# shanice-l/gdrnpp_bop2022

Hardware: AMD Instinct MI355X
Metric: ROIs/sec (GDRNPP fwd + PnP + depth refine), 256x256 crops (higher is better)
Workload: dtype f32

## Files before the change

gdrnpp_bop2022_amd/csrc/capi.hip:

```cpp
#include "gemm_split.hpp"
#include <cstring>
#include <atomic>
#include <mutex>

namespace gdrnpp {
static thread_local char g_err[512] = "";
void set_error(const char* fmt, ...) {
  va_list ap;
  va_start(ap, fmt);
  vsnprintf(g_err, sizeof(g_err), fmt, ap);
  va_end(ap);
}
void* shim_scratch(size_t bytes) {
  static thread_local void* block = nullptr;
  static thread_local size_t cap = 0;
  static thread_local int block_dev = -1;
  int dev = 0;
  hipError_t e = hipGetDevice(&dev);
  if (e != hipSuccess) { set_error("hipGetDevice: %s", hipGetErrorString(e)); return nullptr; }
  if (block && block_dev == dev && cap >= bytes) return block;
  if (block) { (void)hipFree(block); block = nullptr; cap = 0; }
  const size_t want = bytes < ((size_t)1 << 20) ? ((size_t)1 << 20) : bytes + (bytes >> 2);
  e = hipMalloc(&block, want);
  if (e != hipSuccess) { block = nullptr; set_error("hipMalloc(%zu): %s", want, hipGetErrorString(e)); return nullptr; }
  cap = want; block_dev = dev;
  return block;
}
int ensure_dynamic_lds(const void* kernel, int bytes) {
  struct Entry { const void* fn; int dev, bytes; };
  static std::mutex mu;
  static Entry table[128];
  static int n = 0;
  int dev = 0;
  GDRNPP_HIP_TRY(hipGetDevice(&dev));
  std::lock_guard<std::mutex> lock(mu);
  Entry* e = nullptr;
  for (int i = 0; i < n; ++i)
    if (table[i].fn == kernel && table[i].dev == dev) e = &table[i];
  if (e && e->bytes >= bytes) return 0;
  GDRNPP_HIP_TRY(hipFuncSetAttribute(kernel, hipFuncAttributeMaxDynamicSharedMemorySize, bytes));
  if (e) e->bytes = bytes;
  else if (n < 128) table[n++] = Entry{kernel, dev, bytes};
  return 0;
}
static std::atomic<int> g_opt_glds{1}, g_opt_mi4{-1}, g_opt_pipe{3}, g_opt_panel{4}, g_opt_big_tiles{256}, g_opt_dw_tile{-1}, g_opt_splitk_small{1}, g_opt_mlp_fused_pipe{1}, g_opt_dw_lds_w{1}, g_opt_dw_lds_pad{0}, g_opt_upconv_lowres{1}, g_opt_dw_specialise{1};
int option_split_gemm_glds() { return g_opt_glds; }
int option_split_gemm_pipe() { return g_opt_pipe; }
int option_split_gemm_mi4() { return g_opt_mi4; }
int option_split_gemm_panel() { return g_opt_panel; }
int option_split_gemm_big_tiles() { return g_opt_big_tiles; }
int option_dwconv_tile() { return g_opt_dw_tile; }
int option_splitk_small_tiles() { return g_opt_splitk_small; }
int option_mlp_fused_pipe() { return g_opt_mlp_fused_pipe; }
int option_dwconv_lds_w() { return g_opt_dw_lds_w; }
int option_dwconv_lds_pad() { return g_opt_dw_lds_pad; }
int option_dwconv_specialise() { return g_opt_dw_specialise; }
}

namespace {
template <int WIDTH>
__global__ void stream_read_kernel(const float* __restrict__ p, size_t n, float* __restrict__ out) {
  float acc = 0.f;
  const size_t stride = (size_t)gridDim.x * blockDim.x;
  if (WIDTH == 4) {
    const float4* q = reinterpret_cast<const float4*>(p);
    for (size_t i = (size_t)blockIdx.x * blockDim.x + threadIdx.x; i < n / 4; i += stride) {
      const float4 v = q[i];
      acc += (v.x + v.y) + (v.z + v.w);
    }
  } else {
    for (size_t i = (size_t)blockIdx.x * blockDim.x + threadIdx.x; i < n; i += stride) acc += p[i];
  }
  for (int off = 32; off >= 1; off >>= 1) acc += __shfl_xor(acc, off, 64);
  if ((threadIdx.x & 63) == 0) atomicAdd(out + blockIdx.x, acc);
}
__global__ void spin_kernel(long long ticks) {
  const long long t0 = wall_clock64();
  while (wall_clock64() - t0 < ticks) __builtin_amdgcn_s_sleep(8);
}
}

extern "C" {
int gdrnpp_debug_spin(int micros, void* stream) {
  GDRNPP_REQUIRE(micros >= 1 && micros <= 1000000, GDRNPP_EINVAL, "gdrnpp_debug_spin: micros must be in [1, 1000000]");
  int dev = 0, khz = 0;
  GDRNPP_HIP_TRY(hipGetDevice(&dev));
  GDRNPP_HIP_TRY(hipDeviceGetAttribute(&khz, hipDeviceAttributeWallClockRate, dev));
  if (khz <= 0) khz = 100000;
  hipLaunchKernelGGL(spin_kernel, dim3(1), dim3(64), 0, (hipStream_t)stream, (long long)micros * khz / 1000);
  return gdrnpp::check_launch("gdrnpp_debug_spin");
}
int gdrnpp_debug_stream_read(const float* p, size_t n, int lane_bytes, float* out_blocks, int blocks, void* stream) {
  GDRNPP_REQUIRE(p && out_blocks && n > 0 && blocks > 0 && (lane_bytes == 4 || lane_bytes == 16), GDRNPP_EINVAL,
                 "gdrnpp_debug_stream_read: bad arguments");
  if (lane_bytes == 16)
    hipLaunchKernelGGL(stream_read_kernel<4>, dim3(blocks), dim3(256), 0, (hipStream_t)stream, p, n, out_blocks);
  else
    hipLaunchKernelGGL(stream_read_kernel<1>, dim3(blocks), dim3(256), 0, (hipStream_t)stream, p, n, out_blocks);
  return gdrnpp::check_launch("gdrnpp_debug_stream_read");
}
int gdrnpp_copy_d2d(void* dst, const void* src, size_t bytes, void* stream) {
  if (bytes == 0) return 0;
  GDRNPP_REQUIRE(dst && src, GDRNPP_EINVAL, "gdrnpp_copy_d2d: null pointer");
  GDRNPP_HIP_TRY(hipMemcpyAsync(dst, src, bytes, hipMemcpyDeviceToDevice, (hipStream_t)stream));
  return 0;
}
int gdrnpp_set_option(const char* name, int value) {
  GDRNPP_REQUIRE(name, GDRNPP_EINVAL, "gdrnpp_set_option: null name");
  if (!strcmp(name, "split_gemm_glds")) { gdrnpp::g_opt_glds = value != 0; return 0; }
  if (!strcmp(name, "split_gemm_pipe")) { gdrnpp::g_opt_pipe = value == 3 ? 3 : (value != 0 ? 2 : 0); return 0; }
  if (!strcmp(name, "split_gemm_panel")) { gdrnpp::g_opt_panel = value < 2 ? 0 : (value > 64 ? 64 : value); return 0; }
  if (!strcmp(name, "split_gemm_big_tiles")) { gdrnpp::g_opt_big_tiles = value < 1 ? 1 : value; return 0; }
  if (!strcmp(name, "splitk_small_tiles")) { gdrnpp::g_opt_splitk_small = value != 0; return 0; }
  if (!strcmp(name, "dwconv_tile")) { gdrnpp::g_opt_dw_tile = (value >= 0 && value <= 2) ? value : -1; return 0; }
  if (!strcmp(name, "mlp_fused_pipe")) { gdrnpp::g_opt_mlp_fused_pipe = value != 0; return 0; }
  if (!strcmp(name, "dwconv_lds_w")) { gdrnpp::g_opt_dw_lds_w = value != 0; return 0; }
  if (!strcmp(name, "dwconv_specialise")) { gdrnpp::g_opt_dw_specialise = value != 0; return 0; }
  if (!strcmp(name, "dwconv_lds_pad")) { gdrnpp::g_opt_dw_lds_pad = value < 0 ? 0 : (value > 112 * 1024 ? 112 * 1024 : value); return 0; }
  if (!strcmp(name, "split_gemm_mi4")) { gdrnpp::g_opt_mi4 = value < 0 ? -1 : (value != 0); return 0; }
  if (!strcmp(name, "upconv_lowres")) { gdrnpp::g_opt_upconv_lowres = value != 0; return 0; }
  gdrnpp::set_error("gdrnpp_set_option: unknown option '%s'", name);
  return GDRNPP_EINVAL;
}
int gdrnpp_get_option(const char* name, int* value) {
  GDRNPP_REQUIRE(name && value, GDRNPP_EINVAL, "gdrnpp_get_option: null pointer");
  static const struct { const char* name; std::atomic<int>* opt; } table[] = {
      {"split_gemm_glds", &gdrnpp::g_opt_glds},       {"split_gemm_pipe", &gdrnpp::g_opt_pipe},
      {"split_gemm_panel", &gdrnpp::g_opt_panel},     {"split_gemm_big_tiles", &gdrnpp::g_opt_big_tiles},
      {"splitk_small_tiles", &gdrnpp::g_opt_splitk_small}, {"dwconv_tile", &gdrnpp::g_opt_dw_tile},
      {"mlp_fused_pipe", &gdrnpp::g_opt_mlp_fused_pipe}, {"dwconv_lds_w", &gdrnpp::g_opt_dw_lds_w},
      {"dwconv_lds_pad", &gdrnpp::g_opt_dw_lds_pad},  {"split_gemm_mi4", &gdrnpp::g_opt_mi4},
      {"upconv_lowres", &gdrnpp::g_opt_upconv_lowres}, {"dwconv_specialise", &gdrnpp::g_opt_dw_specialise}};
  for (const auto& e : table)
    if (!strcmp(name, e.name)) { *value = e.opt->load(); return 0; }
  gdrnpp::set_error("gdrnpp_get_option: unknown option '%s'", name);
  return GDRNPP_EINVAL;
}
int gdrnpp_version(void) { return 110;  }
const char* gdrnpp_last_error(void) { return gdrnpp::g_err; }
}
```

gdrnpp_bop2022_amd/csrc/common.hpp:

```cpp
#pragma once
#include <hip/hip_runtime.h>
#include <cstdio>
#include <cstdarg>
#include <cstdlib>
#include "../../include/gdrnpp_hip.h"

namespace gdrnpp {

void set_error(const char* fmt, ...);

inline int check_launch(const char* what) {
  hipError_t e = hipGetLastError();
  if (e != hipSuccess) {
    set_error("%s: %s", what, hipGetErrorString(e));
    return (int)e;
  }
  return 0;
}

#define GDRNPP_REQUIRE(cond, code, ...) \
  do {                                  \
    if (!(cond)) {                      \
      gdrnpp::set_error(__VA_ARGS__);   \
      return (code);                    \
    }                                   \
  } while (0)

#define GDRNPP_HIP_TRY(expr)                                        \
  do {                                                              \
    hipError_t _e = (expr);                                         \
    if (_e != hipSuccess) {                                         \
      gdrnpp::set_error("%s: %s", #expr, hipGetErrorString(_e));    \
      return (int)_e;                                               \
    }                                                               \
  } while (0)

constexpr int kWave = 64;

__device__ __forceinline__ float gelu_erf(float x) {
  const float u = fminf(fabsf(x), 5.9f);
  float q = -2.7721912374545354e-06f;
  q = fmaf(q, u, 3.862218727590516e-05f);
  q = fmaf(q, u, -0.00018255332543049008f);
  q = fmaf(q, u, -0.000145858692121692f);
  q = fmaf(q, u, 0.007075459696352482f);
  q = fmaf(q, u, -0.052505023777484894f);
  q = fmaf(q, u, -0.45920491218566895f);
  q = fmaf(q, u, -1.1511057615280151f);
  q = fmaf(q, u, -1.0f);
  const float r = fmaf(-u, __builtin_amdgcn_exp2f(q), fmaxf(x, 0.f));
  return x != x ? x : r;
}

void* shim_scratch(size_t bytes);
int ensure_dynamic_lds(const void* kernel, int bytes);

int option_split_gemm_glds();
int option_split_gemm_mi4();
int option_splitk_small_tiles();
int option_mlp_fused_pipe();
int option_dwconv_tile();
int option_dwconv_lds_w();
int option_dwconv_specialise();
int option_dwconv_lds_pad();

}
```

gdrnpp_bop2022_amd/csrc/gemm_split2_pipe.hip:

```cpp
#include "split2_common.hpp"

namespace {

using namespace gdrnpp::split2;

constexpr int NA = 3;
constexpr int A_STAGE_B = 256 * BK * 4;
constexpr int W2_TILE_SLOTS = 2 * KB * BN;
constexpr int W2_TILE_B = W2_TILE_SLOTS * 16;
constexpr int NB = 4;
constexpr int NJ = 4;
constexpr int LDS_BYTES = NA * A_STAGE_B + NB * W2_TILE_B;

__device__ int g_split2_range_word;

template <bool APRE>
struct HalfSplit2T {
  float x[APRE ? 1 : 8];
  unsigned h[4], l[4];

  template <int S>
  __device__ __forceinline__ void step() {
    if constexpr (APRE) {
    } else if constexpr (S < 2) {
      h[2 * S] = cvt_pk_f16(x[4 * S], x[4 * S + 1]);
      h[2 * S + 1] = cvt_pk_f16(x[4 * S + 2], x[4 * S + 3]);
    } else if constexpr (S < 6) {
      constexpr int p = S - 2;
      x[2 * p] = residual<0>(x[2 * p], h[p]);
      x[2 * p + 1] = residual<1>(x[2 * p + 1], h[p]);
    } else {
      constexpr int q = S - 6;
      l[2 * q] = cvt_pk_f16(x[4 * q], x[4 * q + 1]);
      l[2 * q + 1] = cvt_pk_f16(x[4 * q + 2], x[4 * q + 3]);
    }
  }
  __device__ __forceinline__ void load(const uint4* lds, int slot0, int slot1) {
    if constexpr (APRE) {
      const uint4 a = lds[slot0], b = lds[slot1];
      h[0] = a.x; h[1] = a.y; h[2] = a.z; h[3] = a.w;
      l[0] = b.x; l[1] = b.y; l[2] = b.z; l[3] = b.w;
    } else {
      const float4 a = __builtin_bit_cast(float4, lds[slot0]), b = __builtin_bit_cast(float4, lds[slot1]);
      x[0] = a.x; x[1] = a.y; x[2] = a.z; x[3] = a.w;
      x[4] = b.x; x[5] = b.y; x[6] = b.z; x[7] = b.w;
    }
  }
  template <int SPLIT>
  __device__ __forceinline__ f16x8 frag() const {
    const unsigned* s = SPLIT == 0 ? h : l;
    return __builtin_bit_cast(f16x8, make_uint4(s[0], s[1], s[2], s[3]));
  }
};

__global__ void pack_weight2_kernel(const float* __restrict__ W, uint4* __restrict__ packed, int N, int K) {
  const long i = (long)blockIdx.x * blockDim.x + threadIdx.x;
  const int kbs = K / 8;
  unsigned* trailer = reinterpret_cast<unsigned*>(packed + (size_t)(N / BN) * (K / BK) * W2_TILE_SLOTS);
  const int e = weight_exp(trailer[0]);
  const float sc = __builtin_ldexpf(1.f, e);
  if (i == 0) {
    trailer[1] = __float_as_uint(__builtin_ldexpf(1.f, -e));
    trailer[2] = __float_as_uint(sc);
    trailer[3] = 0u;
  }
  if (i >= (long)N * kbs) return;
  const int n = (int)(i / kbs), kb_g = (int)(i % kbs);
  const float4 v0 = *reinterpret_cast<const float4*>(W + (size_t)n * K + kb_g * 8);
  const float4 v1 = *reinterpret_cast<const float4*>(W + (size_t)n * K + kb_g * 8 + 4);
  const float x[8] = {v0.x * sc, v0.y * sc, v0.z * sc, v0.w * sc, v1.x * sc, v1.y * sc, v1.z * sc, v1.w * sc};
  unsigned h[4], l[4];
#pragma unroll
  for (int p = 0; p < 4; ++p) {
    h[p] = cvt_pk_f16(x[2 * p], x[2 * p + 1]);
    const f16x2 hv = __builtin_bit_cast(f16x2, h[p]);
    l[p] = cvt_pk_f16(x[2 * p] - (float)hv[0], x[2 * p + 1] - (float)hv[1]);
  }
  const int tn = n / BN, row = n % BN, tk = kb_g / KB, kb = kb_g % KB;
  uint4* img = packed + ((size_t)tn * (K / BK) + tk) * W2_TILE_SLOTS;
  img[(0 * KB + kb) * BN + row] = make_uint4(h[0], h[1], h[2], h[3]);
  img[(1 * KB + kb) * BN + row] = make_uint4(l[0], l[1], l[2], l[3]);
}

template <int EPI, int CONV, bool GNS, bool APRE = false>
__global__ __launch_bounds__(256, 2) void gemm_split2_pipe_kernel(const float* __restrict__ A, const uint4* __restrict__ Wp,
                                                                  const float* __restrict__ bias,
                                                                  const float* __restrict__ gamma,
                                                                  const float* __restrict__ resid, float* __restrict__ C,
                                                                  int M, int N, int K, ConvGeom cg, int panel, GnStats gn, int* range_flag, int c_rows) {
  static_assert(!APRE || CONV == 0, "f16x2-rows A: linear form only");
  using HalfSplit2 = HalfSplit2T<APRE>;
  constexpr int NS = 6 * NJ;
  constexpr int SB = 19;
  extern __shared__ uint4 smem[];
  const int tid = threadIdx.x, lane = tid & 63;
  const int wave = __builtin_amdgcn_readfirstlane(tid >> 6);
  const int ntn = N / BN;
  const TileMN tile = tile_coords(xcd_tile_id(), ntn, panel, M);
  const int tile_n = tile.n, m0 = tile.m * 256, n0 = tile_n * BN;
  const int nk = K / BK;
  const unsigned lds0 = lds_addr(smem);
  const float wsc = reinterpret_cast<const float*>(Wp + (size_t)(N / BN) * nk * W2_TILE_SLOTS)[1];

  const int prow = lane >> 2, pq = lane & 3;
  unsigned aoff[4];
  const float* ap[4];
  unsigned okmask[4];
  int cpt = 1;
#pragma unroll
  for (int c = 0; c < 4; ++c) {
    const int lrow = wave * 64 + c * 16 + prow;
    const int q = pq ^ ((lrow >> 2) & 3);
    const int arow = min(m0 + lrow, M - 1);
    if constexpr (CONV == 1) {
      const int img = arow / (cg.H * cg.W), pp = arow - img * (cg.H * cg.W);
      const int iy = pp / cg.W, ix = pp - iy * cg.W;
      ap[c] = A + ((size_t)arow) * cg.C + q * 4;
      unsigned mk = 0;
#pragma unroll
      for (int t = 0; t < 9; ++t) {
        const int dy = t / 3 - 1, dx = t % 3 - 1;
        if ((unsigned)(iy + dy) < (unsigned)cg.H && (unsigned)(ix + dx) < (unsigned)cg.W) mk |= 1u << t;
      }
      okmask[c] = mk;
      aoff[c] = 0;
    } else if constexpr (CONV == 2) {
      const int img = arow / (cg.OH * cg.OW), pp = arow - img * (cg.OH * cg.OW);
      const int iy = (pp / cg.OW) * cg.stride, ix = (pp % cg.OW) * cg.stride;
      ap[c] = A + (((size_t)img * cg.H + iy) * cg.W + ix) * cg.C + q * 4;
      const int ntaps = K / cg.C;
      unsigned mk = 0;
      for (int t = 0; t < ntaps; ++t) {
        const int ky = t / cg.KW, dy = ky - cg.pad, dx = t - ky * cg.KW - cg.pad;
        if ((unsigned)(iy + dy) < (unsigned)cg.H && (unsigned)(ix + dx) < (unsigned)cg.W) mk |= 1u << t;
      }
      okmask[c] = mk;
      aoff[c] = 0;
    } else {
      aoff[c] = (unsigned)arow * (unsigned)(K * 4) + (unsigned)(q * 16);
      ap[c] = nullptr;
      okmask[c] = 0;
    }
  }
  if constexpr (CONV) cpt = cg.C / BK;
  const int ntaps = CONV == 1 ? 9 : (CONV == 2 ? K / cg.C : 1), ckw = CONV == 1 ? 3 : cg.KW, cpad = CONV == 1 ? 1 : cg.pad;
  const unsigned boff = (unsigned)((wave * 2) * 64 + lane) * 16u;
  const char* const wbase = reinterpret_cast<const char*>(Wp + (size_t)tile_n * nk * W2_TILE_SLOTS);
  const unsigned ldsA = lds0 + (unsigned)(wave * 4) * 1024u;
  const unsigned ldsB = lds0 + (unsigned)(NA * A_STAGE_B) + (unsigned)(wave * 2) * 1024u;

  auto dma_a = [&](int kt, unsigned sb, auto cc) {
    constexpr int c = decltype(cc)::value;
    if constexpr (CONV) {
      GDRNPP_CONV_KTILE(kt, cpt, ntaps);
      const int c0 = chunk * BK;
      const int ky = tap / ckw, dy = ky - cpad, dx = tap - ky * ckw - cpad;
      const long off = ((long)dy * cg.W + dx) * cg.C + c0;
      const bool ok = (okmask[c] >> tap) & 1u;
      dma_v(ok ? (const void*)(ap[c] + off) : (const void*)g_zero_page, ldsA + sb + c * 1024u);
    } else {
      dma_s(aoff[c], reinterpret_cast<const char*>(A) + (size_t)kt * (BK * 4), ldsA + sb + c * 1024u);
    }
  };
  auto dma_b = [&](int kt, unsigned sb, auto cc) {
    constexpr int c = decltype(cc)::value;
    int wkt = kt;
    if constexpr (CONV) {
      GDRNPP_CONV_KTILE(kt, cpt, ntaps);
      wkt = tap * cpt + chunk;
    }
    dma_s(boff, wbase + ((size_t)wkt * W2_TILE_B + c * 1024), ldsB + sb + (unsigned)(c * 1024));
  };

  f32x16 acc[2][NJ];
#pragma unroll
  for (int i = 0; i < 2; ++i)
#pragma unroll
    for (int j = 0; j < NJ; ++j)
#pragma unroll
      for (int r = 0; r < 16; ++r) acc[i][j][r] = 0.f;

  const int frow = lane & 31, fk = lane >> 5;
  const int lrow0 = wave * 64 + frow, g0 = (lrow0 >> 2) & 3;
  const int aslot0 = 4 * lrow0 + ((2 * fk) ^ g0), aslot1 = 4 * lrow0 + ((2 * fk + 1) ^ g0);
  const uint4* const sA = smem;
  const uint4* const sBf = smem + NA * (A_STAGE_B / 16) + fk * BN + frow;

  auto load_half = [&](HalfSplit2& hs, int stage, int half) {
    hs.load(sA + stage * (A_STAGE_B / 16) + half * 128, aslot0, aslot1);
  };

  auto bslot = [](int P, int J) { return P * KB * BN + J * 32; };

  [[maybe_unused]] float ssq[4] = {0.f, 0.f, 0.f, 0.f};

  auto ktile = [&](int kt, HalfSplit2 (&cur)[2], HalfSplit2 (&nxt)[2], f16x8 (&fbL)[NJ], f16x8 (&fbH)[NJ], auto odd_, int sa1, int sa2,
                   int sa_wr) {
    constexpr int ODD = decltype(odd_)::value;
    const uint4* const b = sBf + (kt & 3) * (W2_TILE_B / 16);
    const uint4* const bn = sBf + ((kt + 1) & 3) * (W2_TILE_B / 16);
    const int kt_b = min(kt + 2, nk - 1), kt_a = min(kt + NA, nk - 1);
    const unsigned sb_wr = (unsigned)(((kt + 2) & 3) * W2_TILE_B), sa_wr_b = (unsigned)(sa_wr * A_STAGE_B);
    static_for<0, NS>([&](auto s_) {
      constexpr int S = decltype(s_)::value;
      constexpr int G = S / (2 * NJ), I = (S % (2 * NJ)) / NJ, J = S % NJ;
      const f16x8 fa = (G == 1) ? cur[I].template frag<1>() : cur[I].template frag<0>();
      const f16x8 fb = (G == 0) ? fbL[J] : fbH[J];
      acc[I][J] = __builtin_amdgcn_mfma_f32_32x32x16_f16(fa, fb, acc[I][J], 0, 0, 0);
#ifndef GDRNPP2_TIMING_NO_DMA
      if constexpr (S % 2 == 0 && S < 4) dma_b(kt_b, sb_wr, std::integral_constant<int, S / 2>{});
      if constexpr (S % 2 == 0 && S >= 4 && S < 12) dma_a(kt_a, sa_wr_b, std::integral_constant<int, (S - 4) / 2>{});
#endif
#ifndef GDRNPP2_TIMING_NO_BREAD
      if constexpr (S % 2 == 1 && S < NJ) {
        constexpr int j0 = S - 1;
        fbH[j0] = __builtin_bit_cast(f16x8, b[bslot(0, j0)]);
        fbH[j0 + 1] = __builtin_bit_cast(f16x8, b[bslot(0, j0 + 1)]);
      }
#endif
#ifndef GDRNPP2_NO_RANGE_CHECK
      {
        constexpr int rc[4] = {0, 2, 11, 12};
        if constexpr (S == rc[0]) { ssq[2] = sumsq2(cur[1].h[0], ssq[2]); ssq[3] = sumsq2(cur[1].h[1], ssq[3]); }
        if constexpr (S == rc[1]) { ssq[2] = sumsq2(cur[1].h[2], ssq[2]); ssq[3] = sumsq2(cur[1].h[3], ssq[3]); }
        if constexpr (S == rc[2]) { ssq[0] = sumsq2(cur[0].h[0], ssq[0]); ssq[1] = sumsq2(cur[0].h[1], ssq[1]); }
        if constexpr (S == rc[3]) { ssq[0] = sumsq2(cur[0].h[2], ssq[0]); ssq[1] = sumsq2(cur[0].h[3], ssq[1]); }
      }
#endif
      constexpr int S1 = 13;
      if constexpr (S == S1 - 4) load_half(nxt[1], sa1, 1);
#ifndef GDRNPP2_TIMING_NO_SPLIT
      if constexpr (S >= 3 && S < 11) nxt[0].template step<S - 3>();
      if constexpr (S >= S1 && S < S1 + 8) nxt[1].template step<S - S1>();
#else
      if constexpr (S == 3) { nxt[0].h[0] = __float_as_uint(nxt[0].x[0]); nxt[0].h[1] = __float_as_uint(nxt[0].x[1]); nxt[0].h[2] = __float_as_uint(nxt[0].x[2]); nxt[0].h[3] = __float_as_uint(nxt[0].x[3]);
                              nxt[0].l[0] = __float_as_uint(nxt[0].x[4]); nxt[0].l[1] = __float_as_uint(nxt[0].x[5]); nxt[0].l[2] = __float_as_uint(nxt[0].x[6]); nxt[0].l[3] = __float_as_uint(nxt[0].x[7]); }
      if constexpr (S == S1) { nxt[1].h[0] = __float_as_uint(nxt[1].x[0]); nxt[1].h[1] = __float_as_uint(nxt[1].x[1]); nxt[1].h[2] = __float_as_uint(nxt[1].x[2]); nxt[1].h[3] = __float_as_uint(nxt[1].x[3]);
                               nxt[1].l[0] = __float_as_uint(nxt[1].x[4]); nxt[1].l[1] = __float_as_uint(nxt[1].x[5]); nxt[1].l[2] = __float_as_uint(nxt[1].x[6]); nxt[1].l[3] = __float_as_uint(nxt[1].x[7]); }
#endif
      if constexpr (S == SB) {
#ifndef GDRNPP2_TIMING_NO_SYNC
        wait_vmcnt<4>();
        __builtin_amdgcn_s_waitcnt(0xc07f);
        if constexpr (ODD) __builtin_amdgcn_s_barrier();
#endif
      }
      constexpr int SL = APRE ? SB + 1 : SB;
#ifndef GDRNPP2_TIMING_NO_BREAD
      if constexpr (S > SL && S <= SL + NJ / 2) {
        constexpr int j0 = 2 * (S - SL - 1);
        fbL[j0] = __builtin_bit_cast(f16x8, bn[bslot(1, j0)]);
        fbL[j0 + 1] = __builtin_bit_cast(f16x8, bn[bslot(1, j0 + 1)]);
      }
#endif
      if constexpr (S == (APRE ? SB + 1 : SB + NJ / 2 + 1)) load_half(cur[0], sa2, 0);
      __builtin_amdgcn_sched_barrier(0);
    });
  };

  HalfSplit2 f0[2], f1[2];
  f16x8 fbL[NJ], fbH[NJ];
  static_for<0, 4>([&](auto c) { dma_a(0, 0u, c); });
  static_for<0, 2>([&](auto c) { dma_b(0, 0u, c); });
  static_for<0, 2>([&](auto c) { dma_b(min(1, nk - 1), (unsigned)W2_TILE_B, c); });
  static_for<0, 4>([&](auto c) { dma_a(min(1, nk - 1), (unsigned)A_STAGE_B, c); });
  static_for<0, 4>([&](auto c) { dma_a(min(2, nk - 1), 2u * A_STAGE_B, c); });
  wait_vmcnt<4>();
  __builtin_amdgcn_s_barrier();
  load_half(f0[0], 0, 0);
  load_half(f0[1], 0, 1);
  static_for<0, 8>([&](auto s) { f0[0].template step<decltype(s)::value>(); f0[1].template step<decltype(s)::value>(); });
#pragma unroll
  for (int j = 0; j < NJ; ++j) fbL[j] = __builtin_bit_cast(f16x8, sBf[bslot(1, j)]);
  load_half(f1[0], 1, 0);

  int sa = 0;
  for (int kt = 0; kt < nk; kt += 2) {
    const int sa1 = sa + 1 == NA ? 0 : sa + 1, sa2 = sa1 + 1 == NA ? 0 : sa1 + 1, sa3 = sa2 + 1 == NA ? 0 : sa2 + 1;
    ktile(kt, f0, f1, fbL, fbH, std::integral_constant<int, 0>{}, sa1, sa2, sa);
    ktile(kt + 1, f1, f0, fbL, fbH, std::integral_constant<int, 1>{}, sa2, sa3, sa1);
    sa = sa2;
  }
  wait_vmcnt<0>();
  __builtin_amdgcn_s_waitcnt(0xc07f);
  __builtin_amdgcn_s_barrier();

  bool bad = false;
#define EPI_TILES_M 2
#define EPI_HALVES (NJ / 2)
#define EPI_ACC(i, j) acc[i][j]
#define EPI_ROW0 m0 + wave * 64
#define EPI_COL0 n0
#define EPI_BIAS bias
#define EPI_STAGE smem
#define EPI_STAGE_BYTES (NA * A_STAGE_B)
#define EPI_SCALE wsc
#define EPI_GN gn
#define EPI_RANGE_BAD bad
#include "split_epilogue_body.hpp"
  bool small = false;
#ifndef GDRNPP2_NO_RANGE_CHECK
  {
    float s0 = ssq[0] + ssq[1], s1 = ssq[2] + ssq[3];
    s0 += __shfl_xor(s0, 32, 64);
    s1 += __shfl_xor(s1, 32, 64);
    const float thr = (float)K * 0x1p-8f;
    small = (s0 > 0.f && s0 < thr) || (s1 > 0.f && s1 < thr);
    bad |= !(s0 < __builtin_inff()) || !(s1 < __builtin_inff());
  }
#endif
  const int word = (__builtin_amdgcn_ballot_w64(bad) != 0 ? GDRNPP_SPLIT2_NONFINITE : 0) |
                   (__builtin_amdgcn_ballot_w64(small) != 0 ? GDRNPP_SPLIT2_SMALL_ROWS : 0);
  if (word && lane == 0) atomicOr(range_flag ? range_flag : &g_split2_range_word, word);
}

template <int EPI, int CONV, bool GNS, bool APRE = false>
int launch_kernel(const float* A, const uint4* Wp, const float* bias, const float* gamma, const float* resid, float* C, int M, int N,
                  int K, ConvGeom cg, int panel, GnStats gn, int* range_flag, hipStream_t st, const char* what, int c_rows = 0) {
  const int rc = gdrnpp::ensure_dynamic_lds((const void*)gemm_split2_pipe_kernel<EPI, CONV, GNS, APRE>, LDS_BYTES);
  if (rc) return rc;
  const long tiles = (long)((M + 255) / 256) * (N / BN);
  GDRNPP_REQUIRE(tiles < (1l << 30), GDRNPP_ELIMIT, "%s: grid too large", what);
  hipLaunchKernelGGL((gemm_split2_pipe_kernel<EPI, CONV, GNS, APRE>), dim3((unsigned)tiles), dim3(256), LDS_BYTES, st, A, Wp, bias, gamma,
                     resid, C, M, N, K, cg, panel, gn, range_flag, c_rows);
  return gdrnpp::check_launch(what);
}

template <int EPI, int CONV, bool GNS>
int launch_one(const float* A, const uint4* Wp, const float* bias, const float* gamma, const float* resid, float* C, int M, int N,
               int K, ConvGeom cg, int panel, GnStats gn, int* range_flag, hipStream_t st, const char* what, int a_rows = 0, int c_rows = 0) {
  if constexpr (CONV == 0 && EPI != EPI_BIAS) {
    if (a_rows) return launch_kernel<EPI, CONV, GNS, true>(A, Wp, bias, gamma, resid, C, M, N, K, cg, panel, gn, range_flag, st, what, c_rows);
  }
  return launch_kernel<EPI, CONV, GNS>(A, Wp, bias, gamma, resid, C, M, N, K, cg, panel, gn, range_flag, st, what, c_rows);
}

}

extern "C" size_t gdrnpp_pack_weight_f16x2_bytes(int N, int K) {
  return (N > 0 && K > 0) ? (size_t)N * (size_t)K * 4 + 16 : 0;
}

extern "C" int gdrnpp_pack_weight_f16x2(const float* W, void* packed, int N, int K, void* stream) {
  GDRNPP_REQUIRE(W && packed, GDRNPP_EINVAL, "gdrnpp_pack_weight_f16x2: null pointer");
  GDRNPP_REQUIRE(N > 0 && K > 0 && N % BN == 0 && K % 32 == 0, GDRNPP_ELIMIT,
                 "gdrnpp_pack_weight_f16x2: N=%d K=%d must be multiples of %d/32", N, K, BN);
  hipStream_t st = (hipStream_t)stream;
  unsigned* trailer = reinterpret_cast<unsigned*>(reinterpret_cast<uint4*>(packed) + (size_t)(N / BN) * (K / BK) * W2_TILE_SLOTS);
  GDRNPP_HIP_TRY(hipMemsetAsync(trailer, 0, 16, st));
  const long n = (long)N * K;
  hipLaunchKernelGGL(amax_kernel, dim3((unsigned)min((n + 1023) / 1024, 1024l)), dim3(256), 0, st, W, n, trailer);
  const long threads = (long)N * (K / 8);
  hipLaunchKernelGGL(pack_weight2_kernel, dim3((unsigned)((threads + 255) / 256)), dim3(256), 0, st, W, (uint4*)packed, N, K);
  hipLaunchKernelGGL(weight_rows_range_kernel, dim3((unsigned)N), dim3(256), 0, st, W, trailer, trailer + 3, K);
  return gdrnpp::check_launch("gdrnpp_pack_weight_f16x2");
}

extern "C" int gdrnpp_linear_f32_split2_rows(const float* A, const void* W_packed, const float* bias, const float* gamma,
                                             const float* resid, float* C, int M, int N, int K, int epilogue, int rows,
                                             int* range_flag, void* stream) {
  GDRNPP_REQUIRE(A && W_packed && C, GDRNPP_EINVAL, "gdrnpp_linear_f32_split2: null pointer");
  GDRNPP_REQUIRE(M > 0 && N > 0 && K > 0 && N % BN == 0 && K % 32 == 0, GDRNPP_ELIMIT,
                 "gdrnpp_linear_f32_split2: N=%d K=%d must be multiples of %d/32 (M=%d is free)", N, K, BN, M);
  GDRNPP_REQUIRE((unsigned long long)M * (unsigned long long)K * 4ull < (1ull << 32), GDRNPP_ELIMIT,
                 "gdrnpp_linear_f32_split2: M*K*4 must stay below 4 GiB (32-bit lane offsets)");
  GDRNPP_REQUIRE(epilogue >= 0 && epilogue <= 2, GDRNPP_EINVAL, "gdrnpp_linear_f32_split2: epilogue=%d", epilogue);
  GDRNPP_REQUIRE(epilogue != EPI_SCALE_RES || (gamma && resid), GDRNPP_EINVAL,
                 "gdrnpp_linear_f32_split2: scale+residual epilogue needs gamma and resid");
  GDRNPP_REQUIRE((rows & ~(GDRNPP_A_F16X2_ROWS | GDRNPP_C_F16X2_ROWS)) == 0, GDRNPP_EINVAL, "gdrnpp_linear_f32_split2_rows: rows=%d", rows);
  GDRNPP_REQUIRE(!(rows & GDRNPP_C_F16X2_ROWS) || epilogue != EPI_SCALE_RES, GDRNPP_EINVAL,
                 "gdrnpp_linear_f32_split2_rows: the scale+residual epilogue writes fp32");
  GDRNPP_REQUIRE(!(rows & GDRNPP_A_F16X2_ROWS) || epilogue != EPI_BIAS, GDRNPP_ELIMIT,
                 "gdrnpp_linear_f32_split2_rows: an f16x2-rows A needs the GELU or the scale+residual epilogue (the two MLP layers)");
  const int panel = (N / BN >= 8 && (long)N * K * 4 > (2l << 20)) ? gdrnpp::option_split_gemm_panel() : 0;
  const ConvGeom cg{0, 0, 0, 0, 0, 0, 0, 0, 0};
  const GnStats gn{nullptr, 0, 0};
  hipStream_t st = (hipStream_t)stream;
  const uint4* Wp = (const uint4*)W_packed;
  const char* what = "gdrnpp_linear_f32_split2";
  const int ar = rows & GDRNPP_A_F16X2_ROWS, cr = (rows & GDRNPP_C_F16X2_ROWS) ? 1 : 0;
  return with_epilogue(epilogue, [&](auto epi) {
    return launch_one<decltype(epi)::value, 0, false>(A, Wp, bias, gamma, resid, C, M, N, K, cg, panel, gn, range_flag, st, what, ar, cr);
  });
}

extern "C" int gdrnpp_linear_f32_split2(const float* A, const void* W_packed, const float* bias, const float* gamma,
                                        const float* resid, float* C, int M, int N, int K, int epilogue, int* range_flag,
                                        void* stream) {
  return gdrnpp_linear_f32_split2_rows(A, W_packed, bias, gamma, resid, C, M, N, K, epilogue, 0, range_flag, stream);
}

extern "C" int gdrnpp_conv3x3_f32_split2(const float* x_nhwc, const void* W_packed, const float* bias, float* y_nhwc,
                                         double* gn_partials, int n_img, int H, int W, int Cin, int Cout, int groups, int epilogue,
                                         int* range_flag, void* stream) {
  GDRNPP_REQUIRE(x_nhwc && W_packed && y_nhwc, GDRNPP_EINVAL, "gdrnpp_conv3x3_f32_split2: null pointer");
  GDRNPP_REQUIRE(n_img > 0 && H > 0 && W > 0 && H < 32768 && W < 32768 && Cin > 0 && Cout > 0, GDRNPP_EINVAL,
                 "gdrnpp_conv3x3_f32_split2: bad shape");
  const long M = (long)n_img * H * W;
  GDRNPP_REQUIRE(M < (1l << 31) && Cout % BN == 0 && Cin % 32 == 0, GDRNPP_ELIMIT,
                 "gdrnpp_conv3x3_f32_split2: Cout=%d Cin=%d must be multiples of %d/32", Cout, Cin, BN);
  GDRNPP_REQUIRE(epilogue == EPI_BIAS || epilogue == EPI_GELU, GDRNPP_EINVAL, "gdrnpp_conv3x3_f32_split2: epilogue=%d", epilogue);
  const ConvGeom cg{H, W, Cin, H, W, 3, 1, 1, 0};
  hipStream_t st = (hipStream_t)stream;
  const uint4* Wp = (const uint4*)W_packed;
  const char* what = "gdrnpp_conv3x3_f32_split2";
  if (gn_partials) {
    GDRNPP_REQUIRE(epilogue == EPI_BIAS && (H * W) % 256 == 0 && groups > 0 && Cout == 8 * groups, GDRNPP_ELIMIT,
                   "gdrnpp_conv3x3_f32_split2: GroupNorm statistics need the plain epilogue, H*W %% 256 == 0 and 8 channels per group "
                   "(H*W=%d Cout=%d groups=%d)", H * W, Cout, groups);
    return launch_one<EPI_BIAS, 1, true>(x_nhwc, Wp, bias, nullptr, nullptr, y_nhwc, (int)M, Cout, 9 * Cin, cg, 0,
                                         GnStats{gn_partials, groups, (H * W) / 256}, range_flag, st, what);
  }
  const GnStats gn{nullptr, 0, 0};
  if (epilogue == EPI_GELU)
    return launch_one<EPI_GELU, 1, false>(x_nhwc, Wp, bias, nullptr, nullptr, y_nhwc, (int)M, Cout, 9 * Cin, cg, 0, gn, range_flag, st, what);
  return launch_one<EPI_BIAS, 1, false>(x_nhwc, Wp, bias, nullptr, nullptr, y_nhwc, (int)M, Cout, 9 * Cin, cg, 0, gn, range_flag, st, what);
}

extern "C" int gdrnpp_conv2d_f32_split2(const float* x_nhwc, const void* W_packed, const float* bias, float* y_nhwc, int n_img,
                                        int H, int W, int Cin, int Cout, int KH, int KW, int stride, int pad, int epilogue,
                                        int* range_flag, void* stream) {
  GDRNPP_REQUIRE(x_nhwc && W_packed && y_nhwc, GDRNPP_EINVAL, "gdrnpp_conv2d_f32_split2: null pointer");
  ConvShape sh;
  if (const int rc = check_conv_shape("gdrnpp_conv2d_f32_split2", n_img, H, W, Cin, Cout, KH, KW, stride, pad, 32, &sh)) return rc;
  if (KH == 3 && KW == 3 && stride == 1 && pad == 1)
    return gdrnpp_conv3x3_f32_split2(x_nhwc, W_packed, bias, y_nhwc, nullptr, n_img, H, W, Cin, Cout, 0, epilogue, range_flag, stream);
  const int OH = sh.OH, OW = sh.OW;
  const long M = sh.M;
  GDRNPP_REQUIRE(epilogue == EPI_BIAS || epilogue == EPI_GELU, GDRNPP_EINVAL, "gdrnpp_conv2d_f32_split2: epilogue=%d", epilogue);
  const ConvGeom cg{H, W, Cin, OH, OW, KW, stride, pad, 0};
  const GnStats gn{nullptr, 0, 0};
  hipStream_t st = (hipStream_t)stream;
  const uint4* Wp = (const uint4*)W_packed;
  const char* what = "gdrnpp_conv2d_f32_split2";
  if (epilogue == EPI_GELU)
    return launch_one<EPI_GELU, 2, false>(x_nhwc, Wp, bias, nullptr, nullptr, y_nhwc, (int)M, Cout, KH * KW * Cin, cg, 0, gn, range_flag, st, what);
  return launch_one<EPI_BIAS, 2, false>(x_nhwc, Wp, bias, nullptr, nullptr, y_nhwc, (int)M, Cout, KH * KW * Cin, cg, 0, gn, range_flag, st, what);
}

extern "C" int gdrnpp_split2_range_word(int* flag, int reset, void* stream) {
  GDRNPP_REQUIRE(flag, GDRNPP_EINVAL, "gdrnpp_split2_range_word: null pointer");
  hipStream_t st = (hipStream_t)stream;
  int v = 0;
  GDRNPP_HIP_TRY(hipMemcpyFromSymbolAsync(&v, HIP_SYMBOL(g_split2_range_word), sizeof(int), 0, hipMemcpyDeviceToHost, st));
  GDRNPP_HIP_TRY(hipStreamSynchronize(st));
  if (reset && v) {
    const int zero = 0;
    GDRNPP_HIP_TRY(hipMemcpyToSymbolAsync(HIP_SYMBOL(g_split2_range_word), &zero, sizeof(int), 0, hipMemcpyHostToDevice, st));
    GDRNPP_HIP_TRY(hipStreamSynchronize(st));
  }
  *flag = v;
  return 0;
}
```

Before: 5749.

## Add sliding-window conv3x3 kernel that stages input rows once per channel chunk

Adds a dedicated 3x3 stride-1 convolution kernel for image widths 16/32/64. It DMAs a window of 256 output rows plus a one-row halo per channel chunk into LDS and reuses it across all nine taps, instead of gathering im2col tiles for every tap. Edge columns are zeroed in registers, and weight tiles are streamed through a four-deep ring. The new path is on by default behind a new option. It adds a large hand-scheduled kernel with two windows' worth of LDS, and correctness risk at row and image boundaries.

```diff
diff --git a/gdrnpp_bop2022_amd/csrc/capi.hip b/gdrnpp_bop2022_amd/csrc/capi.hip
--- a/gdrnpp_bop2022_amd/csrc/capi.hip
+++ b/gdrnpp_bop2022_amd/csrc/capi.hip
@@ -43,7 +43,7 @@
   else if (n < 128) table[n++] = Entry{kernel, dev, bytes};
   return 0;
 }
-static std::atomic<int> g_opt_glds{1}, g_opt_mi4{-1}, g_opt_pipe{3}, g_opt_panel{4}, g_opt_big_tiles{256}, g_opt_dw_tile{-1}, g_opt_splitk_small{1}, g_opt_mlp_fused_pipe{1}, g_opt_dw_lds_w{1}, g_opt_dw_lds_pad{0}, g_opt_upconv_lowres{1}, g_opt_dw_specialise{1};
+static std::atomic<int> g_opt_glds{1}, g_opt_mi4{-1}, g_opt_pipe{3}, g_opt_panel{4}, g_opt_big_tiles{256}, g_opt_dw_tile{-1}, g_opt_splitk_small{1}, g_opt_mlp_fused_pipe{1}, g_opt_dw_lds_w{1}, g_opt_dw_lds_pad{0}, g_opt_upconv_lowres{1}, g_opt_dw_specialise{1}, g_opt_conv3x3_window{1};
 int option_split_gemm_glds() { return g_opt_glds; }
 int option_split_gemm_pipe() { return g_opt_pipe; }
 int option_split_gemm_mi4() { return g_opt_mi4; }
@@ -55,6 +55,7 @@
 int option_dwconv_lds_w() { return g_opt_dw_lds_w; }
 int option_dwconv_lds_pad() { return g_opt_dw_lds_pad; }
 int option_dwconv_specialise() { return g_opt_dw_specialise; }
+int option_conv3x3_window() { return g_opt_conv3x3_window; }
 }
 
 namespace {
@@ -119,6 +120,7 @@
   if (!strcmp(name, "dwconv_lds_pad")) { gdrnpp::g_opt_dw_lds_pad = value < 0 ? 0 : (value > 112 * 1024 ? 112 * 1024 : value); return 0; }
   if (!strcmp(name, "split_gemm_mi4")) { gdrnpp::g_opt_mi4 = value < 0 ? -1 : (value != 0); return 0; }
   if (!strcmp(name, "upconv_lowres")) { gdrnpp::g_opt_upconv_lowres = value != 0; return 0; }
+  if (!strcmp(name, "conv3x3_window")) { gdrnpp::g_opt_conv3x3_window = value != 0; return 0; }
   gdrnpp::set_error("gdrnpp_set_option: unknown option '%s'", name);
   return GDRNPP_EINVAL;
 }
@@ -130,7 +132,8 @@
       {"splitk_small_tiles", &gdrnpp::g_opt_splitk_small}, {"dwconv_tile", &gdrnpp::g_opt_dw_tile},
       {"mlp_fused_pipe", &gdrnpp::g_opt_mlp_fused_pipe}, {"dwconv_lds_w", &gdrnpp::g_opt_dw_lds_w},
       {"dwconv_lds_pad", &gdrnpp::g_opt_dw_lds_pad},  {"split_gemm_mi4", &gdrnpp::g_opt_mi4},
-      {"upconv_lowres", &gdrnpp::g_opt_upconv_lowres}, {"dwconv_specialise", &gdrnpp::g_opt_dw_specialise}};
+      {"upconv_lowres", &gdrnpp::g_opt_upconv_lowres}, {"dwconv_specialise", &gdrnpp::g_opt_dw_specialise},
+      {"conv3x3_window", &gdrnpp::g_opt_conv3x3_window}};
   for (const auto& e : table)
     if (!strcmp(name, e.name)) { *value = e.opt->load(); return 0; }
   gdrnpp::set_error("gdrnpp_get_option: unknown option '%s'", name);
diff --git a/gdrnpp_bop2022_amd/csrc/common.hpp b/gdrnpp_bop2022_amd/csrc/common.hpp
--- a/gdrnpp_bop2022_amd/csrc/common.hpp
+++ b/gdrnpp_bop2022_amd/csrc/common.hpp
@@ -62,6 +62,7 @@
 int option_dwconv_tile();
 int option_dwconv_lds_w();
 int option_dwconv_specialise();
+int option_conv3x3_window();
 int option_dwconv_lds_pad();
 
 }
diff --git a/gdrnpp_bop2022_amd/csrc/gemm_split2_pipe.hip b/gdrnpp_bop2022_amd/csrc/gemm_split2_pipe.hip
--- a/gdrnpp_bop2022_amd/csrc/gemm_split2_pipe.hip
+++ b/gdrnpp_bop2022_amd/csrc/gemm_split2_pipe.hip
@@ -333,6 +333,221 @@
     if (a_rows) return launch_kernel<EPI, CONV, GNS, true>(A, Wp, bias, gamma, resid, C, M, N, K, cg, panel, gn, range_flag, st, what, c_rows);
   }
   return launch_kernel<EPI, CONV, GNS>(A, Wp, bias, gamma, resid, C, M, N, K, cg, panel, gn, range_flag, st, what, c_rows);
+}
+
+constexpr int WIN_B = (256 + 2 * 64) * 64;
+constexpr int WIN_LDS_BYTES = 2 * WIN_B + NB * W2_TILE_B;
+static_assert(WIN_LDS_BYTES <= LDS_BYTES, "two workgroups per CU");
+
+__device__ __forceinline__ void zero_raw(HalfSplit2T<false>& hs, bool z) {
+#pragma unroll
+  for (int i = 0; i < 8; ++i) hs.x[i] = z ? 0.f : hs.x[i];
+}
+
+template <int EPI, int IW, bool GNS>
+__global__ __launch_bounds__(256, 2) void conv3x3_window_kernel(const float* __restrict__ A, const uint4* __restrict__ Wp,
+                                                                const float* __restrict__ bias, float* __restrict__ C, int M, int N,
+                                                                ConvGeom cg, GnStats gn, int* range_flag) {
+  using HalfSplit2 = HalfSplit2T<false>;
+  constexpr int NS = 6 * NJ, SB = 19, S1 = 13;
+  constexpr int NPIECES = (256 + 2 * IW) / 16;
+  constexpr int NPW = (NPIECES + 3) / 4;
+  constexpr int WPMAX = 255 + 2 * IW;
+  static_assert(NPW <= 6, "the pieces of a window go out in k-tiles 0 .. 5 of the chunk before");
+  extern __shared__ uint4 smem[];
+  const int tid = threadIdx.x, lane = tid & 63;
+  const int wave = __builtin_amdgcn_readfirstlane(tid >> 6);
+  const int ntn = N / BN;
+  const TileMN tile = tile_coords(xcd_tile_id(), ntn, 0, M);
+  const int tile_n = tile.n, m0 = tile.m * 256, n0 = tile_n * BN;
+  const int cpt = cg.C / BK, nk = 9 * cpt, K = 9 * cg.C;
+  const unsigned lds0 = lds_addr(smem);
+  const float wsc = reinterpret_cast<const float*>(Wp + (size_t)(N / BN) * nk * W2_TILE_SLOTS)[1];
+  const float* const gamma = nullptr;
+  const float* const resid = nullptr;
+  constexpr int c_rows = 0;
+
+  const int y0 = (m0 % (cg.H * IW)) / IW;
+  const unsigned woff = (unsigned)(lane >> 2) * (unsigned)(cg.C * 4) + (unsigned)(((lane & 3) ^ ((lane >> 4) & 3)) * 16);
+  const unsigned zoff = (unsigned)(lane & 3) * 16u;
+  auto dma_win = [&](int chunk, unsigned wb, int j) {
+    const int p = j * 4 + wave;
+    if (p < NPIECES) {
+      const int y = y0 - 1 + (16 * p) / IW;
+      const unsigned dst = lds0 + wb + (unsigned)p * 1024u;
+      if ((unsigned)y < (unsigned)cg.H)
+        dma_s(woff, A + ((long)m0 - IW + 16 * p) * cg.C + chunk * BK, dst);
+      else
+        dma_s(zoff, g_zero_page, dst);
+    }
+  };
+  const unsigned boff = (unsigned)((wave * 2) * 64 + lane) * 16u;
+  const char* const wbase = reinterpret_cast<const char*>(Wp + (size_t)tile_n * nk * W2_TILE_SLOTS);
+  const unsigned ldsB = lds0 + (unsigned)(2 * WIN_B) + (unsigned)(wave * 2) * 1024u;
+  auto dma_b = [&](int kt, unsigned sb, auto cc) {
+    constexpr int c = decltype(cc)::value;
+    const int chunk = kt / 9, tap = kt - 9 * chunk;
+    dma_s(boff, wbase + ((size_t)(tap * cpt + chunk) * W2_TILE_B + c * 1024), ldsB + sb + (unsigned)(c * 1024));
+  };
+
+  f32x16 acc[2][NJ];
+#pragma unroll
+  for (int i = 0; i < 2; ++i)
+#pragma unroll
+    for (int j = 0; j < NJ; ++j)
+#pragma unroll
+      for (int r = 0; r < 16; ++r) acc[i][j][r] = 0.f;
+
+  const int frow = lane & 31, fk = lane >> 5;
+  const int lrow0 = wave * 64 + frow;
+  const bool edgeL0 = lrow0 % IW == 0, edgeL1 = (lrow0 + 32) % IW == 0;
+  const bool edgeR0 = lrow0 % IW == IW - 1, edgeR1 = (lrow0 + 32) % IW == IW - 1;
+  const uint4* const sBf = smem + 2 * (WIN_B / 16) + fk * BN + frow;
+
+  auto load_half = [&](HalfSplit2& hs, int kt, int half) {
+    const int ktc = min(kt, nk - 1), chunk = ktc / 9, tap = ktc - 9 * chunk, ty = tap / 3;
+    const int toff = IW * ty + (tap - 3 * ty) - 1;
+    const int wp = min(max(lrow0 + half * 32 + toff, 0), WPMAX);
+    const int s0 = 4 * wp + ((2 * fk) ^ ((wp >> 2) & 3));
+    hs.load(smem + (chunk & 1) * (WIN_B / 16), s0, s0 ^ 1);
+  };
+  auto tap_dx = [&](int kt) {
+    const int ktc = min(kt, nk - 1), tap = ktc % 9;
+    return tap % 3 - 1;
+  };
+
+  auto bslot = [](int P, int J) { return P * KB * BN + J * 32; };
+  [[maybe_unused]] float ssq[4] = {0.f, 0.f, 0.f, 0.f};
+
+  auto ktile = [&](int kt, HalfSplit2 (&cur)[2], HalfSplit2 (&nxt)[2], f16x8 (&fbL)[NJ], f16x8 (&fbH)[NJ], auto odd_) {
+    constexpr int ODD = decltype(odd_)::value;
+    const uint4* const b = sBf + (kt & 3) * (W2_TILE_B / 16);
+    const uint4* const bn = sBf + ((kt + 1) & 3) * (W2_TILE_B / 16);
+    const int kt_b = min(kt + 2, nk - 1);
+    const unsigned sb_wr = (unsigned)(((kt + 2) & 3) * W2_TILE_B);
+    const int chunk = kt / 9, tap = kt - 9 * chunk;
+    const bool piece = tap < NPW && tap * 4 + wave < NPIECES && chunk + 1 < cpt;
+    const int dxn = tap_dx(kt + 1);
+    const bool z0 = (dxn < 0 && edgeL0) || (dxn > 0 && edgeR0), z1 = (dxn < 0 && edgeL1) || (dxn > 0 && edgeR1);
+    static_for<0, NS>([&](auto s_) {
+      constexpr int S = decltype(s_)::value;
+      constexpr int G = S / (2 * NJ), I = (S % (2 * NJ)) / NJ, J = S % NJ;
+      const f16x8 fa = (G == 1) ? cur[I].template frag<1>() : cur[I].template frag<0>();
+      const f16x8 fb = (G == 0) ? fbL[J] : fbH[J];
+      acc[I][J] = __builtin_amdgcn_mfma_f32_32x32x16_f16(fa, fb, acc[I][J], 0, 0, 0);
+      if constexpr (S % 2 == 0 && S < 4) dma_b(kt_b, sb_wr, std::integral_constant<int, S / 2>{});
+      if constexpr (S == 4) {
+        if (piece) dma_win(chunk + 1, (unsigned)(((chunk + 1) & 1) * WIN_B), tap);
+      }
+      if constexpr (S % 2 == 1 && S < NJ) {
+        constexpr int j0 = S - 1;
+        fbH[j0] = __builtin_bit_cast(f16x8, b[bslot(0, j0)]);
+        fbH[j0 + 1] = __builtin_bit_cast(f16x8, b[bslot(0, j0 + 1)]);
+      }
+#ifndef GDRNPP2_NO_RANGE_CHECK
+      {
+        constexpr int rc[4] = {0, 2, 11, 12};
+        if constexpr (S == rc[0]) { ssq[2] = sumsq2(cur[1].h[0], ssq[2]); ssq[3] = sumsq2(cur[1].h[1], ssq[3]); }
+        if constexpr (S == rc[1]) { ssq[2] = sumsq2(cur[1].h[2], ssq[2]); ssq[3] = sumsq2(cur[1].h[3], ssq[3]); }
+        if constexpr (S == rc[2]) { ssq[0] = sumsq2(cur[0].h[0], ssq[0]); ssq[1] = sumsq2(cur[0].h[1], ssq[1]); }
+        if constexpr (S == rc[3]) { ssq[0] = sumsq2(cur[0].h[2], ssq[0]); ssq[1] = sumsq2(cur[0].h[3], ssq[1]); }
+      }
+#endif
+      if constexpr (S == S1 - 4) load_half(nxt[1], kt + 1, 1);
+      if constexpr (S == 3) zero_raw(nxt[0], z0);
+      if constexpr (S == S1) zero_raw(nxt[1], z1);
+      if constexpr (S >= 3 && S < 11) nxt[0].template step<S - 3>();
+      if constexpr (S >= S1 && S < S1 + 8) nxt[1].template step<S - S1>();
+      if constexpr (S == SB) {
+        if (piece) wait_vmcnt<1>(); else wait_vmcnt<0>();
+        __builtin_amdgcn_s_waitcnt(0xc07f);
+        if constexpr (ODD) __builtin_amdgcn_s_barrier();
+      }
+      if constexpr (S > SB && S <= SB + NJ / 2) {
+        constexpr int j0 = 2 * (S - SB - 1);
+        fbL[j0] = __builtin_bit_cast(f16x8, bn[bslot(1, j0)]);
+        fbL[j0 + 1] = __builtin_bit_cast(f16x8, bn[bslot(1, j0 + 1)]);
+      }
+      if constexpr (S == SB + NJ / 2 + 1) load_half(cur[0], kt + 2, 0);
+      __builtin_amdgcn_sched_barrier(0);
+    });
+  };
+
+  HalfSplit2 f0[2], f1[2];
+  f16x8 fbL[NJ], fbH[NJ];
+  for (int j = 0; j < NPW; ++j) dma_win(0, 0u, j);
+  static_for<0, 2>([&](auto c) { dma_b(0, 0u, c); });
+  static_for<0, 2>([&](auto c) { dma_b(1, (unsigned)W2_TILE_B, c); });
+  wait_vmcnt<0>();
+  __builtin_amdgcn_s_barrier();
+  load_half(f0[0], 0, 0);
+  load_half(f0[1], 0, 1);
+  zero_raw(f0[0], edgeL0);
+  zero_raw(f0[1], edgeL1);
+  static_for<0, 8>([&](auto s) { f0[0].template step<decltype(s)::value>(); f0[1].template step<decltype(s)::value>(); });
+#pragma unroll
+  for (int j = 0; j < NJ; ++j) fbL[j] = __builtin_bit_cast(f16x8, sBf[bslot(1, j)]);
+  load_half(f1[0], 1, 0);
+
+  for (int kt = 0; kt < nk; kt += 2) {
+    ktile(kt, f0, f1, fbL, fbH, std::integral_constant<int, 0>{});
+    ktile(kt + 1, f1, f0, fbL, fbH, std::integral_constant<int, 1>{});
+  }
+  wait_vmcnt<0>();
+  __builtin_amdgcn_s_waitcnt(0xc07f);
+  __builtin_amdgcn_s_barrier();
+
+  bool bad = false;
+#define EPI_TILES_M 2
+#define EPI_HALVES (NJ / 2)
+#define EPI_ACC(i, j) acc[i][j]
+#define EPI_ROW0 m0 + wave * 64
+#define EPI_COL0 n0
+#define EPI_BIAS bias
+#define EPI_STAGE smem
+#define EPI_STAGE_BYTES (2 * WIN_B)
+#define EPI_SCALE wsc
+#define EPI_GN gn
+#define EPI_RANGE_BAD bad
+#include "split_epilogue_body.hpp"
+  bool small = false;
+#ifndef GDRNPP2_NO_RANGE_CHECK
+  {
+    float s0 = ssq[0] + ssq[1], s1 = ssq[2] + ssq[3];
+    s0 += __shfl_xor(s0, 32, 64);
+    s1 += __shfl_xor(s1, 32, 64);
+    const float thr = (float)K * 0x1p-8f;
+    small = (s0 > 0.f && s0 < thr) || (s1 > 0.f && s1 < thr);
+    bad |= !(s0 < __builtin_inff()) || !(s1 < __builtin_inff());
+  }
+#endif
+  const int word = (__builtin_amdgcn_ballot_w64(bad) != 0 ? GDRNPP_SPLIT2_NONFINITE : 0) |
+                   (__builtin_amdgcn_ballot_w64(small) != 0 ? GDRNPP_SPLIT2_SMALL_ROWS : 0);
+  if (word && lane == 0) atomicOr(range_flag ? range_flag : &g_split2_range_word, word);
+}
+
+template <int EPI, int IW, bool GNS>
+int launch_window_w(const float* A, const uint4* Wp, const float* bias, float* C, int M, int N, ConvGeom cg, GnStats gn, int* range_flag,
+                    hipStream_t st, const char* what) {
+  const int rc = gdrnpp::ensure_dynamic_lds((const void*)conv3x3_window_kernel<EPI, IW, GNS>, WIN_LDS_BYTES);
+  if (rc) return rc;
+  const long tiles = (long)(M / 256) * (N / BN);
+  GDRNPP_REQUIRE(tiles < (1l << 30), GDRNPP_ELIMIT, "%s: grid too large", what);
+  hipLaunchKernelGGL((conv3x3_window_kernel<EPI, IW, GNS>), dim3((unsigned)tiles), dim3(256), WIN_LDS_BYTES, st, A, Wp, bias, C, M, N, cg, gn,
+                     range_flag);
+  return gdrnpp::check_launch(what);
+}
+
+bool window_form(int H, int W) {
+  return gdrnpp::option_conv3x3_window() && (W == 16 || W == 32 || W == 64) && H % (256 / W) == 0;
+}
+
+template <int EPI, bool GNS>
+int launch_window(const float* A, const uint4* Wp, const float* bias, float* C, int M, int N, ConvGeom cg, GnStats gn, int* range_flag,
+                  hipStream_t st, const char* what) {
+  if (cg.W == 16) return launch_window_w<EPI, 16, GNS>(A, Wp, bias, C, M, N, cg, gn, range_flag, st, what);
+  if (cg.W == 32) return launch_window_w<EPI, 32, GNS>(A, Wp, bias, C, M, N, cg, gn, range_flag, st, what);
+  return launch_window_w<EPI, 64, GNS>(A, Wp, bias, C, M, N, cg, gn, range_flag, st, what);
 }
 
 }
@@ -408,10 +623,16 @@
     GDRNPP_REQUIRE(epilogue == EPI_BIAS && (H * W) % 256 == 0 && groups > 0 && Cout == 8 * groups, GDRNPP_ELIMIT,
                    "gdrnpp_conv3x3_f32_split2: GroupNorm statistics need the plain epilogue, H*W %% 256 == 0 and 8 channels per group "
                    "(H*W=%d Cout=%d groups=%d)", H * W, Cout, groups);
+    if (window_form(H, W))
+      return launch_window<EPI_BIAS, true>(x_nhwc, Wp, bias, y_nhwc, (int)M, Cout, cg, GnStats{gn_partials, groups, (H * W) / 256}, range_flag, st, what);
     return launch_one<EPI_BIAS, 1, true>(x_nhwc, Wp, bias, nullptr, nullptr, y_nhwc, (int)M, Cout, 9 * Cin, cg, 0,
                                          GnStats{gn_partials, groups, (H * W) / 256}, range_flag, st, what);
   }
   const GnStats gn{nullptr, 0, 0};
+  if (window_form(H, W)) {
+    if (epilogue == EPI_GELU) return launch_window<EPI_GELU, false>(x_nhwc, Wp, bias, y_nhwc, (int)M, Cout, cg, gn, range_flag, st, what);
+    return launch_window<EPI_BIAS, false>(x_nhwc, Wp, bias, y_nhwc, (int)M, Cout, cg, gn, range_flag, st, what);
+  }
   if (epilogue == EPI_GELU)
     return launch_one<EPI_GELU, 1, false>(x_nhwc, Wp, bias, nullptr, nullptr, y_nhwc, (int)M, Cout, 9 * Cin, cg, 0, gn, range_flag, st, what);
   return launch_one<EPI_BIAS, 1, false>(x_nhwc, Wp, bias, nullptr, nullptr, y_nhwc, (int)M, Cout, 9 * Cin, cg, 0, gn, range_flag, st, what);
```

Measured after the change: 5844 (median of 6 runs). 1.7% higher.
